# maua-maua-maua/maua

Hardware: AMD Instinct MI355X
Metric: frames/sec (whole node), 1024x1024 StyleGAN2 audio-reactive render (higher is better)
Workload: dtype bf16

## Files before the change

maua_amd/csrc/internal.h:

```cpp
#pragma once
#include "common.h"

namespace maua {

int launch_pack_rgb8(hipStream_t stream, const float* img, uint8_t* out, int B, int H, int W);
template <typename TI, typename TO>
int launch_nchw_to_nhwc(hipStream_t s, const void* x, void* y, int N, int C, int HW, int Cp);
template <typename TI, typename TO>
int launch_nhwc_to_nchw(hipStream_t s, const void* x, void* y, int N, int C, int HW, int Cp);

struct ConvArgs {
  const void* x;
  long x_bstride;
  const void* w;
  const float* s;
  const float* d;
  const float* noise;
  long noise_bstride;
  float noise_strength;
  const float* noise_scale;
  const float* bias;
  void* y;
  int B, H, W, Ci, Co, up;
  int act;
// ... 41 lines not shown

bool lowres_supported(int dtype, int Ci, int Co, int up, int H, int W);
void lowres_workspace(int dtype, int B, int H, int W, int Ci, int Co, int up, size_t* xm_bytes, size_t* ws_bytes);
int launch_modconv_lowres(hipStream_t stream, int dtype, const ConvArgs& a, void* xm, float* ws);

bool gather_conv_supported(int dtype, int Ci, int Co, int H, int W);
size_t gather_conv_workspace(int dtype, int B, int H, int W, int Ci, int Co);
int launch_conv_gather(hipStream_t stream, int dtype, const ConvArgs& a, float* ws);
int gather_conv_check(int dtype, const ConvArgs& a);
int gather_conv_ksplit(int dtype, int B, int H, int W, int Ci, int Co);

struct UnetConvRoute { int kernel; bool wide; int variant; };
UnetConvRoute unet_conv_route(int dtype, int route, int B, int H, int W, int Ci, int Co);

struct HiresArgs {
  const void* x;
  const void* w;
  const float* s;
  const float* d;
  const float* noise;
  long noise_bstride;
  float noise_strength;
  const float* noise_scale;
  const float* bias;
  void* y;
  int B, H, W, Ci, Co, up, act;
  float alpha, gain, clamp;
  const float* rgb_wmod;
  const float* rgb_bias;
  const float* rgb_prev;
  float* rgb_out;
  float rgb_clamp;
  float fir[16];
  uint8_t* rgb8_out;
  int rgb_skip_f32;
};
bool hires_supported(int dtype, int Ci, int Co, int up, int H, int W);
int launch_modconv_hires(hipStream_t stream, const HiresArgs& a, int dtype = MAUA_BF16);
bool upwalk_supported(int dtype, int Ci, int Co, int up, int H, int W);
size_t upwalk_weight_elems(int Co, int Ci);
int launch_upwalk(hipStream_t stream, const HiresArgs& a, int dtype = MAUA_BF16);
int launch_prep_upwalk_weights(hipStream_t stream, const float* w, void* wt, int Co, int Ci, int flip, int dtype = MAUA_BF16);
bool upwalk_fused_supported(int dtype, int Ci, int Cm, int H, int W);
int launch_upwalk_fused(hipStream_t stream, const HiresArgs& up, const HiresArgs& c1, int force_segs = 0, int narrow_ok = 1,
                        int dtype = MAUA_BF16);

int launch_prep_weights(hipStream_t stream, int dtype, const float* w, void* wt, float* wsq, int Co, int Ci, int k,
                        int up, int flip, int Cop, int Cip);
int launch_transpose_flip(hipStream_t stream, const float* w, float* w_t, int Co, int Ci, int kk);
int launch_f32_split_inplace(hipStream_t stream, void* w, long n_floats);

int launch_tconv2(hipStream_t stream, int dtype, const ConvArgs& a);
bool tconv_dma_supported(int dtype, int Ci, int Co, int H, int W);
int launch_tconv_dma(hipStream_t stream, const ConvArgs& a, int dtype = MAUA_BF16);
int launch_tconv_edges(hipStream_t stream, const ConvArgs& a, int dtype = MAUA_BF16);
int launch_prep_tconv_weights(hipStream_t stream, int dtype, const float* w, void* wt, int Co, int Ci, int flip);

struct UpfirArgs {
  const void* t;
  void* y;
  const float* d;
  const float* noise;
  long noise_bstride;
  float noise_strength;
  const float* noise_scale;
  const float* bias;
  const float* out_scale;
  int B, H, W, Co;
  int act;
  float alpha, gain, clamp;
};
int launch_upfir_epilogue(hipStream_t stream, int dtype, const UpfirArgs& a);
bool tconv_fir_supported(int dtype, int Ci, int Co, int H, int W);
int launch_tconv_fir(hipStream_t stream, const ConvArgs& a, const UpfirArgs& u, int dtype = MAUA_BF16, int walk = 1, int force_segs = 0);
size_t prepped_weight_elems(int k, int up, int Cop, int Cip);

struct LayerOperands { const void* x; const void* w; const float* s; const float* d; const float* bias; void* y; int B, H, W, Ci, Co, up; };
struct NoiseOperands { const float* noise; long bstride; float strength; const float* scale; };
struct Epilogue { int act; float alpha, gain, clamp; };
template <typename A>
inline void set_noise_args(A& a, const NoiseOperands& n) {
  a.noise = n.noise; a.noise_bstride = n.bstride; a.noise_strength = n.strength; a.noise_scale = n.scale;
}
template <typename A>
inline void set_epilogue_args(A& a, const Epilogue& e) {
  a.act = e.act; a.alpha = e.alpha; a.gain = e.gain; a.clamp = e.clamp;
}
template <typename A>
inline A layer_args(A a, const LayerOperands& l, const NoiseOperands& n, const Epilogue& e) {
  a.x = l.x; a.w = l.w; a.s = l.s; a.d = l.d; a.bias = l.bias; a.y = l.y;
  a.B = l.B; a.H = l.H; a.W = l.W; a.Ci = l.Ci; a.Co = l.Co; a.up = l.up;
  set_noise_args(a, n);
  set_epilogue_args(a, e);
  return a;
}
template <typename A>
inline void fuse_torgb_args(A& a, const float* wmod, const float* bias, const float* prev, float* out, float clamp, const float* fir16) {
  a.rgb_wmod = wmod; a.rgb_bias = bias; a.rgb_prev = prev; a.rgb_out = out; a.rgb_clamp = clamp;
  for (int i = 0; i < 16; i++) a.fir[i] = fir16[i];
}
inline void pack_u8_args(HiresArgs& a, uint8_t* rgb8_out, bool skip_f32) {
  a.rgb8_out = rgb8_out;
  a.rgb_skip_f32 = skip_f32;
}
inline ConvArgs tconv_args(const void* x, long x_bstride, const void* w, const float* s, void* t, int B, int H, int W, int Ci, int Co) {
  ConvArgs a{};
  a.x = x; a.x_bstride = x_bstride; a.w = w; a.s = s; a.y = t;
// ... 233 lines not shown
```

maua_amd/csrc/modconv_api.hip:

```cpp
#include <algorithm>
#include <cstring>

#include "common.h"
#include "internal.h"
#include "plain_conv.h"

namespace maua {
namespace {

enum { R_LOWRES = 0, R_GENERIC, R_DMA, R_HIRES, R_UPWALK, R_FUSED, R_WALKDONE, R_TFIR, R_TDMA, R_T2, R_UPFIR };

bool is_tconv(int r) { return r == R_TFIR || r == R_TDMA || r == R_T2; }
bool reads_premod(int r) { return r == R_TFIR || r == R_TDMA || r == R_DMA; }

LayerOperands operands(const maua_modconv_desc* d) {
  return LayerOperands{d->x, nullptr, d->s, d->d, d->bias, d->y, d->B, d->H, d->W, d->Ci, d->Co, d->up};
}
NoiseOperands noise_of(const maua_modconv_desc* d) { return NoiseOperands{d->noise, d->noise_bstride, d->noise_strength, d->noise_scale}; }
Epilogue epilogue_of(const maua_modconv_desc* d) { return Epilogue{d->act, d->alpha, d->gain, d->clamp}; }

template <typename A>
A desc_args(const maua_modconv_desc* d) {
  A a = layer_args(A{}, operands(d), noise_of(d), epilogue_of(d));
  if (d->rgb_out) {
// ... 135 lines not shown
  hipStream_t st = ctx->stream;
  if (route == R_UPWALK || route == R_FUSED) {
    if (int rc = launch_prep_upwalk_weights(st, d->w, base + o_w, d->Co, d->Ci, d->flip, dtype)) return rc;
  } else if (is_tconv(route)) {
    if (int rc = launch_prep_tconv_weights(st, dtype, d->w, base + o_w, d->Co, d->Ci, d->flip)) return rc;
  } else if (route != R_UPFIR) {
    if (int rc = launch_prep_weights(st, dtype, d->w, base + o_w, nullptr, d->Co, d->Ci, 3, d->up, d->up == 2 ? d->flip : 0, d->Co, d->Ci))
      return rc;
  }
  if (route == R_FUSED)
    if (int rc = launch_prep_weights(st, dtype, d1->w, base + o_w1, nullptr, d1->Co, d1->Ci, 3, 1, 0, d1->Co, d1->Ci)) return rc;
  const void* x = d->x;
  long x_bstride = d->x_bstride;
  if (reads_premod(route)) {
    if (int rc = launch_premod_nhwc(st, d->x, d->x_bstride, d->s, base + o_xm, d->B, (long)d->H * d->W, d->Ci, dtype)) return rc;
    x = base + o_xm;
    x_bstride = (long)d->H * d->W * d->Ci;
  }
  if (ones_bytes)
    if (int rc = launch_fill_ones(st, (float*)(base + o_ones), (long)d->B * d->Ci)) return rc;
  switch (route) {
    case R_LOWRES:
    case R_GENERIC:
    case R_DMA: {
      ConvArgs a = conv_args(d);
      a.x = x; a.x_bstride = x_bstride; a.w = base + o_w;
      if (route == R_DMA) a.s = nullptr;
      return route == R_LOWRES    ? launch_modconv_lowres(st, dtype, a, base + o_xm, (float*)(base + o_ws))
             : route == R_GENERIC ? launch_modconv3x3(st, dtype, a)
                                  : launch_modconv_dma(st, a, dtype);
    }
    case R_HIRES:
    case R_UPWALK:
    case R_FUSED: {
      HiresArgs a = hires_args(d);
      a.w = base + o_w;
      if (route == R_HIRES) return launch_modconv_hires(st, a, dtype);
      if (route == R_UPWALK) return launch_upwalk(st, a, dtype);
      HiresArgs f = hires_args(d1);
      f.x = nullptr; f.y = nullptr; f.w = base + o_w1;
      a.y = nullptr;
      return launch_upwalk_fused(st, a, f, force_segs, narrow_ok, dtype);
    }
    case R_TFIR:
    case R_TDMA:
    case R_T2: {
      void* t = d->t ? d->t : base + o_t;
      ConvArgs a = tconv_args(d);
      a.x = x; a.x_bstride = x_bstride; a.w = base + o_w; a.y = t;
      if (route != R_T2) a.s = (const float*)(base + o_ones);
      UpfirArgs u = upfir_args(d);
      if (route == R_TFIR) return launch_tconv_fir(st, a, u, dtype, force_segs >= 0, force_segs);
      if (route == R_TDMA) {
        if (int rc = launch_tconv_edges(st, a, dtype)) return rc;
        if (int rc = launch_tconv_dma(st, a, dtype)) return rc;
      } else if (int rc = launch_tconv2(st, dtype, a)) {
        return rc;
      }
      u.t = t;
      return launch_upfir_epilogue(st, dtype, u);
    }
    case R_UPFIR: {
      UpfirArgs u = upfir_args(d);
      u.t = d->x;
      return launch_upfir_epilogue(st, dtype, u);
    }
  }
  return MAUA_OK;
}

extern "C" int maua_torgb_ex(maua_ctx* ctx, const void* x, const float* wmod, const float* bias, const float* prev, float* out, int B,
                             int H, int W, int C, float clamp, int dtype) {
  MAUA_REQUIRE(ctx && x && wmod && bias && out, "maua_torgb_ex: NULL argument");
  MAUA_REQUIRE(B >= 0 && H > 0 && W > 0 && C > 0, "maua_torgb_ex: bad shape");
  MAUA_REQUIRE(!prev || (H % 2 == 0 && W % 2 == 0), "maua_torgb_ex: the skip image needs an even grid");
  RgbArgs r{};
  r.x = x; r.wmod = wmod; r.bias = bias; r.prev = prev; r.out = out; r.B = B; r.H = H; r.W = W; r.C = C; r.clamp = clamp;
  upsample_fir16(r.fir);
  return launch_torgb(ctx->stream, dtype, r);
}
```

maua_amd/csrc/modconv_tconv_dma.hip:

```cpp
#include "common.h"
#include "internal.h"
#include "mma.h"
#include "modconv_tconv.h"

namespace maua {

namespace {

constexpr int PTH = 8, PTW = 32;
constexpr int HW1 = PTW + 1, HPX = (PTH + 1) * HW1;
constexpr int KB = 64;
constexpr int HBUF = HPX * KB;
constexpr int WROWS = 9 * 32;
constexpr int WBUF = WROWS * KB;
constexpr int OFF_H = 2 * WBUF;
constexpr int NW = 4, NT = NW * 64;
constexpr int WJ = (WBUF / 1024 + NW - 1) / NW;
constexpr int HJ = (HPX * 4 + NT - 1) / NT;

}

template <typename F>
__global__ __launch_bounds__(NT, 2) void tconv_dma_kernel(ConvArgs a) {
  constexpr int ES = 128 * 2 + 16, PPP = 16;
  extern __shared__ __attribute__((aligned(1024))) char smem[];
  const unsigned lds0 = __builtin_amdgcn_readfirstlane(lds_off(smem));
  const int tid = threadIdx.x, lane = tid & 63;
  const int wave = __builtin_amdgcn_readfirstlane(tid >> 6);
  const int r = lane & 31, h = lane >> 5;
  const int tiles_x = a.W >> 5, tiles = tiles_x * (a.H >> 3), CB = a.Co >> 5;
  const int cbg = CB < 8 ? CB : 8, n_ts = tiles * a.B, per_group = ((n_ts + 7) >> 3) * 8 * cbg;
  const int L = blockIdx.x, grp = L / per_group, Lg = L - grp * per_group;
  const int xcd = Lg & 7, idx = Lg >> 3;
  const int cb = grp * cbg + idx % cbg, ts = (idx / cbg) * 8 + xcd;
  if (ts >= n_ts) return;
  const int b = ts / tiles, tile = ts - b * tiles;
  const int tyi = tile / tiles_x, txi = tile - tyi * tiles_x;
  const int ty0 = tyi * PTH, tx0 = txi * PTW;
  const char* xb = reinterpret_cast<const char*>(a.x) + (long)b * a.x_bstride * 2;
  const char* wp = reinterpret_cast<const char*>(a.w);

  unsigned hoff[HJ];
#pragma unroll
  for (int j = 0; j < HJ; j++) {
    const int P = (wave + NW * j) * 64 + lane;
    const int hp = P >> 2, q = (P & 3) ^ tconv_swz(hp);
    const int py = (hp * 1986) >> 16;
    const int px = hp - py * HW1;
    const int gy = ty0 - 1 + py, gx = tx0 - 1 + px;
    hoff[j] = 0xffffffffu;
    if (P < HPX * 4) {
      if (gy >= 0 && gx >= 0) {
        hoff[j] = (unsigned)(((gy * a.W + gx) * a.Ci + q * 8) * 2);
      } else {
        *reinterpret_cast<u32x4*>(smem + OFF_H + P * 16) = u32x4{0u, 0u, 0u, 0u};
        *reinterpret_cast<u32x4*>(smem + OFF_H + HBUF + P * 16) = u32x4{0u, 0u, 0u, 0u};
      }
    }
  }
  unsigned woff[WJ];
#pragma unroll
  for (int j = 0; j < WJ; j++) {
    const int ii = wave + NW * j;
    const int R = min(16 * ii + (lane >> 2), WROWS - 1);
    const int k = R >> 5, n = R & 31;
    const int q = (lane & 3) ^ tconv_swz(R);
    woff[j] = (unsigned)((((((kTconvSlot[k] * CB + cb) * 4 + kTconvCls[k]) * 32 + n) * a.Ci) + q * 8) * 2);
  }
#define TD_ISSUE(C_, BUF_)                                                                               \
  {                                                                                                      \
    const char* ws_ = wp + (long)(C_) * KB;                                                              \
    _Pragma("unroll") for (int j = 0; j < WJ; j++)                                                      \
      if (wave + NW * j < WBUF / 1024) dma16_s(ws_, woff[j], lds0 + (BUF_) * WBUF + (wave + NW * j) * 1024); \
    const char* xs_ = xb + (long)(C_) * KB;                                                              \
    _Pragma("unroll") for (int j = 0; j < HJ; j++)                                                      \
      if (hoff[j] != 0xffffffffu) dma16_s(xs_, hoff[j], lds0 + OFF_H + (BUF_) * HBUF + (wave + NW * j) * 1024); \
  }

  const int hp00 = (2 * wave) * HW1 + r;
  const unsigned b0 = (unsigned)(r * KB + ((tconv_swz(r) ^ h) << 4));
#define TD_A(HR_, Q1_, KS_, BUF_)                                                                                              \
  ({                                                                                                                           \
    const int hp_ = hpv + (HR_) * HW1 + (Q1_);                                                                                 \
    *reinterpret_cast<const u32x4*>(smem + ((OFF_H + (BUF_) * HBUF + hp_ * KB + ((tconv_swz(hp_) ^ h) << 4)) ^ ((KS_) << 5))); \
  })
#define TD_B(K_, KS_, BUF_) (*reinterpret_cast<const u32x4*>(smem + (BUF_) * WBUF + (K_) * 32 * KB + (b0 ^ ((KS_) << 5))))

  f32x16 acc[2][4];
#pragma unroll
  for (int R = 0; R < 2; R++)
#pragma unroll
    for (int c = 0; c < 4; c++)
#pragma unroll
      for (int e = 0; e < 16; e++) acc[R][c][e] = 0.f;

  const int n_chunks = a.Ci >> 5;
  TD_ISSUE(0, 0)
  if (n_chunks > 1) TD_ISSUE(1, 1)
  asm volatile("s_waitcnt vmcnt(0)" ::: "memory");
  __syncthreads();
  int hpv = hp00;
#define TD_STEP(KS_, BUF_)                                                                                            \
  {                                                                                                                   \
    u32x4 A00 = TD_A(0, 0, KS_, BUF_), A01 = TD_A(0, 1, KS_, BUF_);                  \
    u32x4 A10 = TD_A(1, 0, KS_, BUF_), A11 = TD_A(1, 1, KS_, BUF_);                                \
    u32x4 A20 = TD_A(2, 0, KS_, BUF_), A21 = TD_A(2, 1, KS_, BUF_);                                \
    {                                                                                                                 \
      const u32x4 B0 = TD_B(0, KS_, BUF_), B1 = TD_B(1, KS_, BUF_), B2 = TD_B(2, KS_, BUF_);                          \
      Mma<F>::step(acc[0][0], B0, A00); Mma<F>::step(acc[1][0], B0, A10);                            \
      Mma<F>::step(acc[0][1], B2, A01); Mma<F>::step(acc[1][1], B2, A11);                   \
      Mma<F>::step(acc[0][0], B1, A01); Mma<F>::step(acc[1][0], B1, A11);                   \
    }                                                                                                                 \
    {                                                                                                                 \
      const u32x4 B3 = TD_B(3, KS_, BUF_), B4 = TD_B(4, KS_, BUF_);                                                   \
      Mma<F>::step(acc[0][2], B4, A10); Mma<F>::step(acc[1][2], B4, A20);                   \
      Mma<F>::step(acc[0][0], B3, A10); Mma<F>::step(acc[1][0], B3, A20);                   \
    }                                                                                                                 \
    {                                                                                                                 \
      const u32x4 B5 = TD_B(5, KS_, BUF_), B6 = TD_B(6, KS_, BUF_), B7 = TD_B(7, KS_, BUF_), B8 = TD_B(8, KS_, BUF_); \
      Mma<F>::step(acc[0][3], B8, A11); Mma<F>::step(acc[1][3], B8, A21);                            \
      Mma<F>::step(acc[0][1], B6, A11); Mma<F>::step(acc[1][1], B6, A21);                                             \
      Mma<F>::step(acc[0][2], B7, A11); Mma<F>::step(acc[1][2], B7, A21);                                             \
      Mma<F>::step(acc[0][0], B5, A11); Mma<F>::step(acc[1][0], B5, A21);                                             \
    }                                                                                                                 \
  }
  for (int c = 0; c < n_chunks; c++) {
    const int buf = c & 1;
    asm volatile("" : "+v"(hpv));
    TD_STEP(0, buf)
    {
      u32x4 A00 = TD_A(0, 0, 1, buf), A01 = TD_A(0, 1, 1, buf), A10 = TD_A(1, 0, 1, buf), A11 = TD_A(1, 1, 1, buf);
      u32x4 A20 = TD_A(2, 0, 1, buf), A21 = TD_A(2, 1, 1, buf);
      const u32x4 B0 = TD_B(0, 1, buf), B1 = TD_B(1, 1, buf), B2 = TD_B(2, 1, buf), B3 = TD_B(3, 1, buf), B4 = TD_B(4, 1, buf);
      const u32x4 B5 = TD_B(5, 1, buf), B6 = TD_B(6, 1, buf), B7 = TD_B(7, 1, buf), B8 = TD_B(8, 1, buf);
      asm volatile("s_waitcnt vmcnt(0)" ::: "memory");
      __syncthreads();
      if (c + 2 < n_chunks) TD_ISSUE(c + 2, buf)
      Mma<F>::step(acc[0][0], B0, A00); Mma<F>::step(acc[1][0], B0, A10);
      Mma<F>::step(acc[0][1], B2, A01); Mma<F>::step(acc[1][1], B2, A11);
      Mma<F>::step(acc[0][0], B1, A01); Mma<F>::step(acc[1][0], B1, A11);
      Mma<F>::step(acc[0][2], B4, A10); Mma<F>::step(acc[1][2], B4, A20);
      Mma<F>::step(acc[0][0], B3, A10); Mma<F>::step(acc[1][0], B3, A20);
      Mma<F>::step(acc[0][3], B8, A11); Mma<F>::step(acc[1][3], B8, A21);
      Mma<F>::step(acc[0][1], B6, A11); Mma<F>::step(acc[1][1], B6, A21);
      Mma<F>::step(acc[0][2], B7, A11); Mma<F>::step(acc[1][2], B7, A21);
      Mma<F>::step(acc[0][0], B5, A11); Mma<F>::step(acc[1][0], B5, A21);
    }
  }
#undef TD_ISSUE
#undef TD_A
#undef TD_B
#undef TD_STEP

  const int Wt = 2 * a.W + 1, Ht = 2 * a.H + 1;
  __syncthreads();
  char* epi = smem;
#pragma unroll
  for (int R = 0; R < 2; R++) {
    const int m = (2 * wave + R) * 32 + r;
#pragma unroll
    for (int c = 0; c < 4; c++)
#pragma unroll
      for (int qd = 0; qd < 4; qd++)
        *reinterpret_cast<uint2*>(epi + m * ES + (c * 32 + 8 * qd + 4 * h) * 2) =
            make_uint2(Fmt16<F>::pack2(acc[R][c][qd * 4 + 0], acc[R][c][qd * 4 + 1]), Fmt16<F>::pack2(acc[R][c][qd * 4 + 2], acc[R][c][qd * 4 + 3]));
  }
  __syncthreads();
  char* yb = reinterpret_cast<char*>(a.y) + (long)b * Ht * Wt * a.Co * 2;
  for (int p = tid; p < PTH * PTW * PPP; p += NT) {
    const int mm = p / PPP, pc = p - mm * PPP;
    const int gy = ty0 + (mm >> 5), gx = tx0 + (mm & 31);
    const int nv = pc * 8, cls = nv >> 5, ch = nv & 31;
    const int oy = 2 * gy + (cls >> 1), ox = 2 * gx + (cls & 1);
    *reinterpret_cast<uint4*>(yb + (((long)oy * Wt + ox) * a.Co + cb * 32 + ch) * 2) =
        *reinterpret_cast<const uint4*>(epi + mm * ES + pc * 16);
  }
}

template <typename F>
__global__ __launch_bounds__(64) void tconv_edges_kernel(ConvArgs a, int row_tiles) {
  const int lane = threadIdx.x, r = lane & 31, h = lane >> 5;
  const int b = blockIdx.y, cb = blockIdx.z, CB = a.Co >> 5;
  const bool row_edge = (int)blockIdx.x < row_tiles;
  const int e0 = (row_edge ? (int)blockIdx.x : (int)blockIdx.x - row_tiles) * 32 + r;
  const uint16_t* xb = reinterpret_cast<const uint16_t*>(a.x) + (long)b * a.x_bstride;
  const uint16_t* wp = reinterpret_cast<const uint16_t*>(a.w);
  long x0 = -1, x1 = -1;
  if (row_edge) {
    if (e0 >= 1 && e0 <= a.W) x0 = ((long)(a.H - 1) * a.W + (e0 - 1)) * a.Ci;
    if (e0 < a.W) x1 = ((long)(a.H - 1) * a.W + e0) * a.Ci;
  } else {
    if (e0 >= 1 && e0 <= a.H - 1) x0 = ((long)(e0 - 1) * a.W + (a.W - 1)) * a.Ci;
    if (e0 < a.H) x1 = ((long)e0 * a.W + (a.W - 1)) * a.Ci;
  }
  const int s1 = row_edge ? 1 : 2, c2 = row_edge ? 1 : 2;
  const uint16_t* w0 = wp + ((((long)0 * CB + cb) * 4 + 0) * 32 + r) * a.Ci + 8 * h;
  const uint16_t* w1 = wp + ((((long)s1 * CB + cb) * 4 + 0) * 32 + r) * a.Ci + 8 * h;
  const uint16_t* w2 = wp + ((((long)s1 * CB + cb) * 4 + c2) * 32 + r) * a.Ci + 8 * h;
  f32x16 acc0, acc1;
#pragma unroll
  for (int e = 0; e < 16; e++) { acc0[e] = 0.f; acc1[e] = 0.f; }
  const u32x4 zero = u32x4{0u, 0u, 0u, 0u};
#pragma unroll 4
  for (int k = 0; k < a.Ci; k += 16) {
    const u32x4 A0 = *reinterpret_cast<const u32x4*>(w0 + k), A1 = *reinterpret_cast<const u32x4*>(w1 + k),
                A2 = *reinterpret_cast<const u32x4*>(w2 + k);
    const u32x4 X0 = x0 >= 0 ? *reinterpret_cast<const u32x4*>(xb + x0 + k + 8 * h) : zero;
    const u32x4 X1 = x1 >= 0 ? *reinterpret_cast<const u32x4*>(xb + x1 + k + 8 * h) : zero;
    Mma<F>::step(acc0, A0, X0);
    Mma<F>::step(acc1, A2, X1);
    Mma<F>::step(acc0, A1, X1);
  }
  const int Wt = 2 * a.W + 1, Ht = 2 * a.H + 1;
  uint16_t* yb = reinterpret_cast<uint16_t*>(a.y) + (long)b * Ht * Wt * a.Co + cb * 32 + 4 * h;
  long o0 = -1, o1 = -1;
  if (row_edge) {
    if (e0 <= a.W) o0 = ((long)(2 * a.H) * Wt + 2 * e0) * a.Co;
    if (e0 < a.W) o1 = ((long)(2 * a.H) * Wt + 2 * e0 + 1) * a.Co;
  } else if (e0 < a.H) {
    o0 = ((long)(2 * e0) * Wt + 2 * a.W) * a.Co;
    o1 = ((long)(2 * e0 + 1) * Wt + 2 * a.W) * a.Co;
  }
#pragma unroll
  for (int qd = 0; qd < 4; qd++) {
    if (o0 >= 0)
      *reinterpret_cast<uint2*>(yb + o0 + 8 * qd) = make_uint2(Fmt16<F>::pack2(acc0[qd * 4], acc0[qd * 4 + 1]), Fmt16<F>::pack2(acc0[qd * 4 + 2], acc0[qd * 4 + 3]));
    if (o1 >= 0)
      *reinterpret_cast<uint2*>(yb + o1 + 8 * qd) = make_uint2(Fmt16<F>::pack2(acc1[qd * 4], acc1[qd * 4 + 1]), Fmt16<F>::pack2(acc1[qd * 4 + 2], acc1[qd * 4 + 3]));
  }
}

int tconv_edges_check(const ConvArgs& a, int dtype) {
  MAUA_REQUIRE(dtype == MAUA_BF16 || dtype == MAUA_F16, "tconv_edges: unsupported dtype");
  MAUA_REQUIRE(a.Ci % 16 == 0 && a.Co % 32 == 0, "tconv_edges: Ci % 16, Co % 32");
  MAUA_REQUIRE(a.B <= 65535 && a.Co / 32 <= 65535, "tconv_edges: grid too large");
  return MAUA_OK;
}
int tconv_dma_check(const ConvArgs& a, int dtype) {
  MAUA_REQUIRE(tconv_dma_supported(dtype, a.Ci, a.Co, a.H, a.W), "tconv_dma: unsupported shape");
  const int tiles = (a.H / PTH) * (a.W / PTW), CB = a.Co / 32, cbg = CB < 8 ? CB : 8;
  MAUA_REQUIRE(CB % cbg == 0, "tconv_dma: channel blocks must split into groups of 8");
  const long n_ts = (long)tiles * a.B, grid = ((n_ts + 7) / 8) * 8 * cbg * (CB / cbg);
  MAUA_REQUIRE(grid < (1L << 31), "tconv_dma: grid too large");
  return MAUA_OK;
}

int launch_tconv_edges(hipStream_t stream, const ConvArgs& a, int dtype) {
  if (int rc = tconv_edges_check(a, dtype)) return rc;
  if (a.B == 0) return MAUA_OK;
  const int row_tiles = (a.W + 1 + 31) / 32, col_tiles = (a.H + 31) / 32;
  if (dtype == MAUA_F16)
    hipLaunchKernelGGL(tconv_edges_kernel<f16_t>, dim3(row_tiles + col_tiles, a.B, a.Co / 32), dim3(64), 0, stream, a, row_tiles);
  else
    hipLaunchKernelGGL(tconv_edges_kernel<bf16_t>, dim3(row_tiles + col_tiles, a.B, a.Co / 32), dim3(64), 0, stream, a, row_tiles);
  MAUA_HIP_CHECK(hipGetLastError());
  return MAUA_OK;
}

bool tconv_dma_supported(int dtype, int Ci, int Co, int H, int W) {
  return (dtype == MAUA_BF16 || dtype == MAUA_F16) && Ci % 32 == 0 && Co % 32 == 0 && H % PTH == 0 && W % PTW == 0 &&
         (long)H * W * Ci * 2 < (1L << 32) && 16L * Co * Ci * 2 < (1L << 32);
}

int launch_tconv_dma(hipStream_t stream, const ConvArgs& a, int dtype) {
  if (int rc = tconv_dma_check(a, dtype)) return rc;
  if (a.B == 0) return MAUA_OK;
  const int tiles = (a.H / PTH) * (a.W / PTW), CB = a.Co / 32, cbg = CB < 8 ? CB : 8;
  const long n_ts = (long)tiles * a.B, grid = ((n_ts + 7) / 8) * 8 * cbg * (CB / cbg);
  const size_t smem = std::max<size_t>((size_t)2 * WBUF + 2 * HBUF, (size_t)PTH * PTW * (128 * 2 + 16));
  if (dtype == MAUA_F16) {
    MAUA_HIP_CHECK(hipFuncSetAttribute((const void*)tconv_dma_kernel<f16_t>, hipFuncAttributeMaxDynamicSharedMemorySize, (int)smem));
    hipLaunchKernelGGL(tconv_dma_kernel<f16_t>, dim3((unsigned)grid), dim3(NT), smem, stream, a);
  } else {
    MAUA_HIP_CHECK(hipFuncSetAttribute((const void*)tconv_dma_kernel<bf16_t>, hipFuncAttributeMaxDynamicSharedMemorySize, (int)smem));
    hipLaunchKernelGGL(tconv_dma_kernel<bf16_t>, dim3((unsigned)grid), dim3(NT), smem, stream, a);
  }
  MAUA_HIP_CHECK(hipGetLastError());
  return MAUA_OK;
}

}
```

maua_amd/csrc/synth.hip:

```cpp
#include <cmath>
#include <cstring>
#include <string>
#include <vector>

#include "common.h"
#include "internal.h"
#include "plain_conv.h"

using namespace maua;

namespace {

struct ConvLayer {
  int block, which;
  int Ci, Co, res, up, w_index;
  int ih = 0, iw = 0;
  int oh = 0, ow = 0;
  int fh = 0, fw = 0;
  float* affine_w = nullptr;
  float* affine_b = nullptr;
  float* bias = nullptr;
  float* noise_const = nullptr;
  float noise_strength = 0.f;
  void* wt = nullptr;
  void* wt_t = nullptr;
  void* wt_h = nullptr;
  float* wsq = nullptr;
  float* s = nullptr;
  float* d = nullptr;
  void* feat = nullptr;
};
struct RgbLayer {
  int block, C, res, w_index;
  int h = 0, w = 0;
  float* affine_w = nullptr;
  float* affine_b = nullptr;
  float* wrgb = nullptr;
  float* bias = nullptr;
  float* s = nullptr;
  float* wmod = nullptr;
};

template <typename T>
int dev_alloc(T** p, size_t n) {
  MAUA_HIP_CHECK(hipMalloc((void**)p, n * sizeof(T)));
  return MAUA_OK;
}

}

struct maua_synth {
  maua_ctx* ctx;
  int res, w_dim, channel_base, channel_max, dtype, nv_compat;
  int nblocks, num_ws;
  size_t esize;
  std::vector<ConvLayer> convs;
  std::vector<RgbLayer> rgbs;
  void* const_x = nullptr;
  int keep_features = 0;
  int lowres = 1;
  int use_hires = 1;
  int upwalk = 2;
  int walk_segs = 0;
  int walk_narrow = 1;
  int fuse_torgb = 1;
  int tconv_up = 1;
  int tconv_fir = 256;
  int tconv_walk = 1;
  const float* nz_scales = nullptr;
  long nz_scale_stride = 0;
  int dma_conv = 1;
  int dual_store = 1;
  int tconv_dma = 1;
  UnitStyles ones;
  void* xm = nullptr;
  void* tbuf = nullptr;
  void* lowres_xm = nullptr;
  float* lowres_ws = nullptr;
  int rs_layer = -1, rs_mode = 0, rs_th = 0, rs_tw = 0, rs_pl = 0, rs_pr = 0, rs_pt = 0, rs_pb = 0, rs_how = 3;
  float rs_value = 0.f;
  float* rs_noise = nullptr;
  void* const_rs = nullptr;
  float* rgb_tmp[2] = {nullptr, nullptr};
  int out_h = 0, out_w = 0;
  int warp_layer[3] = {-1, -1, -1};
  const float* warp_minv[3] = {nullptr, nullptr, nullptr};
  int profile = 0;
  std::vector<hipEvent_t> ev;
  size_t ev_used = 0;
  std::vector<size_t> ev_fwd_start;
  int bcap = 0;
  void* act[2] = {nullptr, nullptr};
  float* img[2] = {nullptr, nullptr};
  StyleLayer* style_table_dev = nullptr;
  float fir[16];
};

static void prof_mark(maua_synth* n) {
  if (!n->profile || n->ev_used >= (1u << 16)) return;
  if (n->ev_used == n->ev.size()) {
    hipEvent_t e;
    if (hipEventCreate(&e) != hipSuccess) return;
    n->ev.push_back(e);
  }
  hipEventRecord(n->ev[n->ev_used++], n->ctx->stream);
}

static int channels_for(int res, int base, int maxc) { return std::min(base / res, maxc); }

static bool lowres_fits(const maua_synth* n, const ConvLayer& c) {
  return lowres_supported(n->dtype, c.Ci, c.Co, c.up, c.ih, c.iw);
}
static bool tconv_dma_fits(const maua_synth* n, const ConvLayer& c) {
  return c.up == 2 && tconv_dma_supported(n->dtype, c.Ci, c.Co, c.ih, c.iw);
}

static void compute_dims(maua_synth* n) {
  int h = 4, w = 4;
  if (n->rs_layer == 0) { h = n->rs_th; w = n->rs_tw; }
  size_t li = 0;
  for (int blk = 0; blk < n->nblocks; blk++) {
    const int nconv = blk == 0 ? 1 : 2;
    for (int k = 0; k < nconv; k++, li++) {
      ConvLayer& c = n->convs[li];
      c.ih = h; c.iw = w;
      c.oh = h * c.up; c.ow = w * c.up;
// ... 355 lines not shown
    MAUA_HIP_CHECK(hipMemcpy(n->rs_noise, fill_noise_host, cnt * sizeof(float), hipMemcpyHostToDevice));
  }
  compute_dims(n);
  free_workspace(n);
  for (size_t i = 0; i < n->convs.size(); i++) {
    ConvLayer& c = n->convs[i];
    if (c.oh != before[i].oh || c.ow != before[i].ow) {
      hipFree(c.noise_const);
      c.noise_const = nullptr;
      MAUA_HIP_CHECK(hipMalloc((void**)&c.noise_const, (size_t)c.oh * c.ow * sizeof(float)));
      MAUA_HIP_CHECK(hipMemset(c.noise_const, 0, (size_t)c.oh * c.ow * sizeof(float)));
    }
  }
  return MAUA_OK;
}

int maua_synth_set_warp(maua_synth* n, int slot, int layer, const float* inv_matrices_dev) {
  MAUA_REQUIRE(n, "maua_synth_set_warp: net is NULL");
  MAUA_REQUIRE(slot >= 0 && slot < 3, "maua_synth_set_warp: slot must be 0..2");
  MAUA_REQUIRE(layer >= 1 && layer <= (int)n->convs.size(), "maua_synth_set_warp: layer must name a synthesis layer (1-based index into layer_names)");
  n->warp_layer[slot] = inv_matrices_dev ? layer : -1;
  n->warp_minv[slot] = inv_matrices_dev;
  return MAUA_OK;
}

int maua_synth_layer_size(const maua_synth* n, int layer, int* h, int* w) {
  MAUA_REQUIRE(n && h && w, "maua_synth_layer_size: NULL argument");
  MAUA_REQUIRE(layer >= -1 && layer < (int)n->convs.size(), "maua_synth_layer_size: no such layer");
  if (layer < 0) { *h = n->out_h; *w = n->out_w; }
  else { *h = n->convs[layer].oh; *w = n->convs[layer].ow; }
  return MAUA_OK;
}

int maua_synth_set_option(maua_synth* n, const char* key, int value) {
  MAUA_REQUIRE(n && key, "maua_synth_set_option: NULL argument");
  if (!strcmp(key, "profile")) {
    n->profile = value;
    n->ev_used = 0;
    n->ev_fwd_start.clear();
    return MAUA_OK;
  }
  if (!strcmp(key, "keep_features")) {
    if (n->keep_features != value) {
      MAUA_HIP_CHECK(hipStreamSynchronize(n->ctx->stream));
      free_workspace(n);
      n->keep_features = value;
    }
    return MAUA_OK;
  }
  static const std::pair<const char*, int maua_synth::*> routing[] = {
      {"lowres", &maua_synth::lowres},         {"use_hires", &maua_synth::use_hires}, {"upwalk", &maua_synth::upwalk},
      {"walk_segs", &maua_synth::walk_segs},   {"walk_narrow", &maua_synth::walk_narrow},
      {"fuse_torgb", &maua_synth::fuse_torgb}, {"tconv_up", &maua_synth::tconv_up},   {"tconv_fir", &maua_synth::tconv_fir},
      {"tconv_walk", &maua_synth::tconv_walk},
      {"tconv_dma", &maua_synth::tconv_dma},   {"dma_conv", &maua_synth::dma_conv},   {"dual_store", &maua_synth::dual_store}};
  for (const auto& o : routing)
    if (!strcmp(key, o.first)) {
      n->*o.second = value;
      return MAUA_OK;
    }
  return fail(std::string("maua_synth_set_option: unknown option ") + key);
}

static thread_local hipMemcpyKind g_load_kind = hipMemcpyHostToDevice;

static int upload(float* dst, const float* host, size_t count, size_t expect, const char* name) {
  if (count != expect)
    return fail(std::string("maua_synth_load: ") + name + ": expected " + std::to_string(expect) + " values, got " +
                std::to_string(count));
  MAUA_HIP_CHECK(hipMemcpy(dst, host, count * sizeof(float), g_load_kind));
  return MAUA_OK;
}

int maua_synth_load(maua_synth* n, const char* name, const float* host, size_t count) {
  MAUA_REQUIRE(n && name && host, "maua_synth_load: NULL argument");
  std::string s(name);
  int blk = -1, pos = 0;
  if (sscanf(name, "bs.%d.%n", &blk, &pos) < 1 || blk < 0 || blk >= n->nblocks || pos == 0)
    return fail("maua_synth_load: unknown parameter name: " + s);
  std::string rest = s.substr(pos);
  hipStream_t st = n->ctx->stream;
  auto check_filter = [&]() -> int {
    if (count != 16) return fail("maua_synth_load: " + s + ": only the 4x4 [1,3,3,1] resample filter is supported");
    const float t[4] = {1, 3, 3, 1};
    for (int u = 0; u < 4; u++)
      for (int v = 0; v < 4; v++)
        if (std::fabs(host[u * 4 + v] - t[u] * t[v] / 64.f) > 1e-6f)
          return fail("maua_synth_load: " + s + ": only the 4x4 [1,3,3,1] resample filter is supported");
    return MAUA_OK;
  };
  if (rest == "resample_filter") return check_filter();
  if (rest == "const") {
    if (blk != 0) return fail("maua_synth_load: only block 0 has a const input");
    int C = n->convs[0].Ci;
    if (count != (size_t)C * 16) return fail("maua_synth_load: bs.0.const: wrong size");
    DevTemp tmp;
    if (int rc = tmp.stage(host, count, g_load_kind)) return rc;
    int rc = n->dtype == MAUA_BF16   ? launch_nchw_to_nhwc<float, bf16_t>(st, tmp.p, n->const_x, 1, C, 16, C)
             : n->dtype == MAUA_F16 ? launch_nchw_to_nhwc<float, f16_t>(st, tmp.p, n->const_x, 1, C, 16, C)
                                    : launch_nchw_to_nhwc<float, float>(st, tmp.p, n->const_x, 1, C, 16, C);
    hipStreamSynchronize(st);
    return rc;
  }
  size_t dot = rest.find('.');
  if (dot == std::string::npos) return fail("maua_synth_load: unknown parameter name: " + s);
  std::string mod = rest.substr(0, dot), par = rest.substr(dot + 1);
  if (mod == "torgb") {
// ... 116 lines not shown
      switch (s.route) {
        case Route::Lowres:
        case Route::Generic:
        case Route::DmaConv1: {
          ConvArgs a = layer_args(ConvArgs{}, li, x, y);
          a.x_bstride = x_bstride;
          a.out_scale = next_s;
          if (s.dual) a.y_scaled = n->xm;
          if (s.rgb) fuse_torgb(a);
          if (s.route == Route::DmaConv1) a.s = nullptr;
          if (int rc = s.route == Route::Lowres    ? launch_modconv_lowres(st, n->dtype, a, n->lowres_xm, n->lowres_ws)
                       : s.route == Route::Generic ? launch_modconv3x3(st, n->dtype, a)
                                                   : launch_modconv_dma(st, a, n->dtype))
            return rc;
          break;
        }
        case Route::Hires:
        case Route::Upwalk:
        case Route::FusedWalk: {
          HiresArgs a = layer_args(HiresArgs{}, li, x, s.skip_store ? nullptr : y);
          if (s.rgb) fuse_torgb(a);
          if (s.rgb8) pack_u8(a);
          if (s.route != Route::Hires) a.w = c.wt_h;
          if (s.route != Route::FusedWalk) {
            if (int rc = s.route == Route::Hires ? launch_modconv_hires(st, a, n->dtype) : launch_upwalk(st, a, n->dtype)) return rc;
            break;
          }
          HiresArgs f = layer_args(HiresArgs{}, li + 1, nullptr, nullptr);
          fuse_torgb(f);
          if (plan.conv[li + 1].rgb8) pack_u8(f);
          if (int rc = launch_upwalk_fused(st, a, f, n->walk_segs, n->walk_narrow, n->dtype)) return rc;
          break;
        }
        case Route::WalkDone:
          break;
        case Route::TconvFir:
        case Route::TconvDma:
        case Route::Tconv2: {
          ConvArgs a = tconv_args(x, x_bstride, c.wt_t, c.s, n->tbuf, B, c.ih, c.iw, c.Ci, c.Co);
          UpfirArgs u = upfir_args(y, c.d, c.bias, next_s, B, c.ih, c.iw, c.Co, layer_noise(li), lrelu_epilogue());
          if (s.src == Src::PremodPass)
            if (int rc = launch_premod_nhwc(st, x, x_bstride, c.s, n->xm, B, (long)c.ih * c.iw, c.Ci, n->dtype)) return rc;
          if (s.src == Src::PremodPass || s.src == Src::Xm) {
            a.x = n->xm;
            a.x_bstride = (long)c.ih * c.iw * c.Ci;
          }
          if (reads_premod(s.route)) a.s = n->ones.p;
          if (s.route == Route::TconvFir) {
            if (int rc = launch_tconv_fir(st, a, u, n->dtype, n->tconv_walk, 0)) return rc;
            prof_mark(n);
            break;
          }
          if (s.route == Route::TconvDma) {
            if (int rc = launch_tconv_edges(st, a, n->dtype)) return rc;
            if (int rc = launch_tconv_dma(st, a, n->dtype)) return rc;
          } else if (int rc = launch_tconv2(st, n->dtype, a)) {
            return rc;
          }
          prof_mark(n);
          u.t = n->tbuf;
          if (int rc = launch_upfir_epilogue(st, n->dtype, u)) return rc;
          break;
        }
      }
      prof_mark(n);
      x = y;
      x_bstride = (long)c.oh * c.ow * c.Co;
      cur ^= 1;
      if (hooked) {
        void* dst = n->keep_features ? c.feat : n->act[cur];
        if (int rc = resize_feat(x, x_bstride, B, c.oh, c.ow, c.Co, dst)) return rc;
        x = dst;
        x_bstride = (long)c.fh * c.fw * c.Co;
        cur ^= 1;
      }
      for (int wsl = 0; wsl < 3; wsl++) {
        if (n->warp_layer[wsl] != (int)li + 1 || !n->warp_minv[wsl]) continue;
        void* dst = n->act[cur];
        if (dst == x) dst = n->act[cur ^ 1];
        if (int rc = launch_warp_affine_nhwc(st, n->dtype, x, dst, n->warp_minv[wsl], B, c.fh, c.fw, c.Co)) return rc;
        if (n->keep_features) {
          MAUA_HIP_CHECK(hipMemcpyAsync(c.feat, dst, (size_t)B * c.fh * c.fw * c.Co * n->esize, hipMemcpyDeviceToDevice, st));
        } else {
          x = dst;
          cur = (dst == n->act[0]) ? 1 : 0;
        }
      }
    }
    if (plan.rgb[blk] != RgbRoute::Fused) {
      const bool hook = plan.rgb[blk] == RgbRoute::Hook;
      RgbArgs r{};
      r.x = x; r.wmod = g.wmod; r.bias = g.bias; r.prev = hook ? nullptr : prev_img;
      r.out = hook ? n->rgb_tmp[0] : rgb_out; r.B = B; r.H = g.h; r.W = g.w; r.C = g.C; r.clamp = 256.f;
      memcpy(r.fir, n->fir, sizeof(r.fir));
      if (int rc = launch_torgb(st, n->dtype, r)) return rc;
      if (hook) {
        const ConvLayer& hc = n->convs[n->rs_layer - 1];
        const int nh = hc.oh, nw = hc.ow;
        ResizeArgs inv{};
        inv.x = n->rgb_tmp[0]; inv.x_bstride = 3L * g.h * g.w; inv.y = n->rgb_tmp[1]; inv.B = B; inv.H = g.h; inv.W = g.w;
        inv.C = 3; inv.oh = nh; inv.ow = nw; inv.mode = n->rs_mode; inv.pl = -n->rs_pl; inv.pt = -n->rs_pt;
        inv.how = MAUA_PAD_CONSTANT; inv.value = 0.f; inv.noise = nullptr;
        if (int rc = launch_resize2d(st, MAUA_F32, false, inv)) return rc;
        const float* native = n->rgb_tmp[1];
        if (prev_img) {
          if (int rc = launch_skip_add(st, n->rgb_tmp[1], prev_img, n->rgb_tmp[0], B, nh, nw, n->fir)) return rc;
          native = n->rgb_tmp[0];
        }
// ... 85 lines not shown
```

Baseline: 4626.

## Fold transposed-conv edge rows and columns into the DMA tconv kernel

Removes the separate tconv_edges kernel launch by having the last-row and last-column tiles of the DMA transposed-conv kernel compute the border outputs with extra MMA steps inside the main K loop. The kernel is templated on an EDGES flag and specialises the loop per tile so interior tiles keep the original instruction stream. Edge waves carry two extra accumulators and write them out directly. This saves one launch and a pass over input and weights per upsampling layer, at the cost of load imbalance on edge tiles and higher register pressure.

```diff
diff --git a/maua_amd/csrc/internal.h b/maua_amd/csrc/internal.h
--- a/maua_amd/csrc/internal.h
+++ b/maua_amd/csrc/internal.h
@@ -117,7 +117,7 @@
 
 int launch_tconv2(hipStream_t stream, int dtype, const ConvArgs& a);
 bool tconv_dma_supported(int dtype, int Ci, int Co, int H, int W);
-int launch_tconv_dma(hipStream_t stream, const ConvArgs& a, int dtype = MAUA_BF16);
+int launch_tconv_dma(hipStream_t stream, const ConvArgs& a, int dtype = MAUA_BF16, bool edges = true);
 int launch_tconv_edges(hipStream_t stream, const ConvArgs& a, int dtype = MAUA_BF16);
 int launch_prep_tconv_weights(hipStream_t stream, int dtype, const float* w, void* wt, int Co, int Ci, int flip);
 
diff --git a/maua_amd/csrc/modconv_api.hip b/maua_amd/csrc/modconv_api.hip
--- a/maua_amd/csrc/modconv_api.hip
+++ b/maua_amd/csrc/modconv_api.hip
@@ -211,8 +211,9 @@
       UpfirArgs u = upfir_args(d);
       if (route == R_TFIR) return launch_tconv_fir(st, a, u, dtype, force_segs >= 0, force_segs);
       if (route == R_TDMA) {
-        if (int rc = launch_tconv_edges(st, a, dtype)) return rc;
-        if (int rc = launch_tconv_dma(st, a, dtype)) return rc;
+        if (force_segs < 0)
+          if (int rc = launch_tconv_edges(st, a, dtype)) return rc;
+        if (int rc = launch_tconv_dma(st, a, dtype, force_segs >= 0)) return rc;
       } else if (int rc = launch_tconv2(st, dtype, a)) {
         return rc;
       }
diff --git a/maua_amd/csrc/modconv_tconv_dma.hip b/maua_amd/csrc/modconv_tconv_dma.hip
--- a/maua_amd/csrc/modconv_tconv_dma.hip
+++ b/maua_amd/csrc/modconv_tconv_dma.hip
@@ -20,7 +20,7 @@
 
 }
 
-template <typename F>
+template <typename F, bool EDGES>
 __global__ __launch_bounds__(NT, 2) void tconv_dma_kernel(ConvArgs a) {
   constexpr int ES = 128 * 2 + 16, PPP = 16;
   extern __shared__ __attribute__((aligned(1024))) char smem[];
@@ -37,6 +37,8 @@
   const int b = ts / tiles, tile = ts - b * tiles;
   const int tyi = tile / tiles_x, txi = tile - tyi * tiles_x;
   const int ty0 = tyi * PTH, tx0 = txi * PTW;
+  const bool row_edge = EDGES && wave == NW - 1 && tyi == (a.H >> 3) - 1;
+  const bool col_edge = EDGES && wave == 0 && txi == tiles_x - 1;
   const char* xb = reinterpret_cast<const char*>(a.x) + (long)b * a.x_bstride * 2;
   const char* wp = reinterpret_cast<const char*>(a.w);
 
@@ -86,7 +88,24 @@
   })
 #define TD_B(K_, KS_, BUF_) (*reinterpret_cast<const u32x4*>(smem + (BUF_) * WBUF + (K_) * 32 * KB + (b0 ^ ((KS_) << 5))))
 
-  f32x16 acc[2][4];
+  const int hpx0 = min(r, PTH) * HW1 + PTW, hpx1 = min(r + 1, PTH) * HW1 + PTW;
+  const unsigned xo0 = (unsigned)(OFF_H + hpx0 * KB + ((tconv_swz(hpx0) ^ h) << 4));
+  const unsigned xo1 = (unsigned)(OFF_H + hpx1 * KB + ((tconv_swz(hpx1) ^ h) << 4));
+#define TD_X(XO_, KS_, BUF_) (*reinterpret_cast<const u32x4*>(smem + (((XO_) + (BUF_) * HBUF) ^ ((KS_) << 5))))
+#define TD_COL(KS_, BUF_)                                                                                \
+  if constexpr (COL) {                                                                                   \
+    const u32x4 X0 = TD_X(xo0, KS_, BUF_);                                                               \
+    u32x4 X1 = TD_X(xo1, KS_, BUF_);                                                                     \
+    if (r >= PTH) X1 = u32x4{0u, 0u, 0u, 0u};                                                            \
+    const u32x4 C0 = TD_B(0, KS_, BUF_), C3 = TD_B(3, KS_, BUF_), C4 = TD_B(4, KS_, BUF_);               \
+    Mma<F>::step(e0, C0, X0); Mma<F>::step(e1, C4, X1); Mma<F>::step(e0, C3, X1);                        \
+  }
+#define TD_ROW(B0_, B1_, B2_, A20_, A21_)                                                                \
+  if constexpr (ROW) { Mma<F>::step(e0, B0_, A20_); Mma<F>::step(e1, B2_, A21_); Mma<F>::step(e0, B1_, A21_); }
+
+  f32x16 acc[2][4], e0, e1;
+#pragma unroll
+  for (int e = 0; e < 16; e++) { e0[e] = 0.f; e1[e] = 0.f; }
 #pragma unroll
   for (int R = 0; R < 2; R++)
 #pragma unroll
@@ -102,6 +121,7 @@
   int hpv = hp00;
 #define TD_STEP(KS_, BUF_)                                                                                            \
   {                                                                                                                   \
+    TD_COL(KS_, BUF_)                                                                                                 \
     u32x4 A00 = TD_A(0, 0, KS_, BUF_), A01 = TD_A(0, 1, KS_, BUF_);                  \
     u32x4 A10 = TD_A(1, 0, KS_, BUF_), A11 = TD_A(1, 1, KS_, BUF_);                                \
     u32x4 A20 = TD_A(2, 0, KS_, BUF_), A21 = TD_A(2, 1, KS_, BUF_);                                \
@@ -110,6 +130,7 @@
       Mma<F>::step(acc[0][0], B0, A00); Mma<F>::step(acc[1][0], B0, A10);                            \
       Mma<F>::step(acc[0][1], B2, A01); Mma<F>::step(acc[1][1], B2, A11);                   \
       Mma<F>::step(acc[0][0], B1, A01); Mma<F>::step(acc[1][0], B1, A11);                   \
+      TD_ROW(B0, B1, B2, A20, A21)                                                                \
     }                                                                                                                 \
     {                                                                                                                 \
       const u32x4 B3 = TD_B(3, KS_, BUF_), B4 = TD_B(4, KS_, BUF_);                                                   \
@@ -124,11 +145,14 @@
       Mma<F>::step(acc[0][0], B5, A11); Mma<F>::step(acc[1][0], B5, A21);                                             \
     }                                                                                                                 \
   }
+  auto k_loop = [&](auto col_, auto row_) __attribute__((always_inline)) {
+  constexpr bool COL = decltype(col_)::value, ROW = decltype(row_)::value;
   for (int c = 0; c < n_chunks; c++) {
     const int buf = c & 1;
     asm volatile("" : "+v"(hpv));
     TD_STEP(0, buf)
     {
+      TD_COL(1, buf)
       u32x4 A00 = TD_A(0, 0, 1, buf), A01 = TD_A(0, 1, 1, buf), A10 = TD_A(1, 0, 1, buf), A11 = TD_A(1, 1, 1, buf);
       u32x4 A20 = TD_A(2, 0, 1, buf), A21 = TD_A(2, 1, 1, buf);
       const u32x4 B0 = TD_B(0, 1, buf), B1 = TD_B(1, 1, buf), B2 = TD_B(2, 1, buf), B3 = TD_B(3, 1, buf), B4 = TD_B(4, 1, buf);
@@ -139,6 +163,7 @@
       Mma<F>::step(acc[0][0], B0, A00); Mma<F>::step(acc[1][0], B0, A10);
       Mma<F>::step(acc[0][1], B2, A01); Mma<F>::step(acc[1][1], B2, A11);
       Mma<F>::step(acc[0][0], B1, A01); Mma<F>::step(acc[1][0], B1, A11);
+      TD_ROW(B0, B1, B2, A20, A21)
       Mma<F>::step(acc[0][2], B4, A10); Mma<F>::step(acc[1][2], B4, A20);
       Mma<F>::step(acc[0][0], B3, A10); Mma<F>::step(acc[1][0], B3, A20);
       Mma<F>::step(acc[0][3], B8, A11); Mma<F>::step(acc[1][3], B8, A21);
@@ -147,12 +172,41 @@
       Mma<F>::step(acc[0][0], B5, A11); Mma<F>::step(acc[1][0], B5, A21);
     }
   }
+  };
+  if (EDGES && row_edge) k_loop(std::false_type{}, std::true_type{});
+  else if (EDGES && col_edge) k_loop(std::true_type{}, std::false_type{});
+  else k_loop(std::false_type{}, std::false_type{});
 #undef TD_ISSUE
 #undef TD_A
 #undef TD_B
 #undef TD_STEP
+#undef TD_X
+#undef TD_COL
+#undef TD_ROW
 
   const int Wt = 2 * a.W + 1, Ht = 2 * a.H + 1;
+  char* yb = reinterpret_cast<char*>(a.y) + (long)b * Ht * Wt * a.Co * 2;
+  if (EDGES && (row_edge || col_edge)) {
+    long o0 = -1, o1 = -1;
+    if (row_edge) {
+      o0 = ((long)(2 * a.H) * Wt + 2 * (tx0 + r)) * a.Co;
+      o1 = o0 + a.Co;
+    } else if (r < PTH) {
+      o0 = ((long)(2 * (ty0 + r)) * Wt + 2 * a.W) * a.Co;
+      o1 = o0 + (long)Wt * a.Co;
+    } else if (r == PTH && ty0 + PTH == a.H) {
+      o0 = ((long)(2 * a.H) * Wt + 2 * a.W) * a.Co;
+    }
+    uint16_t* ye = reinterpret_cast<uint16_t*>(yb) + cb * 32 + 4 * h;
+#pragma unroll
+    for (int qd = 0; qd < 4; qd++) {
+      if (o0 >= 0)
+        *reinterpret_cast<uint2*>(ye + o0 + 8 * qd) = make_uint2(Fmt16<F>::pack2(e0[qd * 4], e0[qd * 4 + 1]), Fmt16<F>::pack2(e0[qd * 4 + 2], e0[qd * 4 + 3]));
+      if (o1 >= 0)
+        *reinterpret_cast<uint2*>(ye + o1 + 8 * qd) = make_uint2(Fmt16<F>::pack2(e1[qd * 4], e1[qd * 4 + 1]), Fmt16<F>::pack2(e1[qd * 4 + 2], e1[qd * 4 + 3]));
+    }
+  }
+
   __syncthreads();
   char* epi = smem;
 #pragma unroll
@@ -166,7 +220,6 @@
             make_uint2(Fmt16<F>::pack2(acc[R][c][qd * 4 + 0], acc[R][c][qd * 4 + 1]), Fmt16<F>::pack2(acc[R][c][qd * 4 + 2], acc[R][c][qd * 4 + 3]));
   }
   __syncthreads();
-  char* yb = reinterpret_cast<char*>(a.y) + (long)b * Ht * Wt * a.Co * 2;
   for (int p = tid; p < PTH * PTW * PPP; p += NT) {
     const int mm = p / PPP, pc = p - mm * PPP;
     const int gy = ty0 + (mm >> 5), gx = tx0 + (mm & 31);
@@ -262,19 +315,26 @@
          (long)H * W * Ci * 2 < (1L << 32) && 16L * Co * Ci * 2 < (1L << 32);
 }
 
-int launch_tconv_dma(hipStream_t stream, const ConvArgs& a, int dtype) {
+template <typename F, bool EDGES>
+static int tconv_dma_launch(hipStream_t stream, const ConvArgs& a, unsigned grid, size_t smem) {
+  MAUA_HIP_CHECK(hipFuncSetAttribute((const void*)tconv_dma_kernel<F, EDGES>, hipFuncAttributeMaxDynamicSharedMemorySize, (int)smem));
+  hipLaunchKernelGGL((tconv_dma_kernel<F, EDGES>), dim3(grid), dim3(NT), smem, stream, a);
+  return MAUA_OK;
+}
+
+int launch_tconv_dma(hipStream_t stream, const ConvArgs& a, int dtype, bool edges) {
+  if (edges)
+    if (int rc = tconv_edges_check(a, dtype)) return rc;
   if (int rc = tconv_dma_check(a, dtype)) return rc;
   if (a.B == 0) return MAUA_OK;
   const int tiles = (a.H / PTH) * (a.W / PTW), CB = a.Co / 32, cbg = CB < 8 ? CB : 8;
-  const long n_ts = (long)tiles * a.B, grid = ((n_ts + 7) / 8) * 8 * cbg * (CB / cbg);
+  const long n_ts = (long)tiles * a.B;
+  const unsigned grid = (unsigned)(((n_ts + 7) / 8) * 8 * cbg * (CB / cbg));
   const size_t smem = std::max<size_t>((size_t)2 * WBUF + 2 * HBUF, (size_t)PTH * PTW * (128 * 2 + 16));
-  if (dtype == MAUA_F16) {
-    MAUA_HIP_CHECK(hipFuncSetAttribute((const void*)tconv_dma_kernel<f16_t>, hipFuncAttributeMaxDynamicSharedMemorySize, (int)smem));
-    hipLaunchKernelGGL(tconv_dma_kernel<f16_t>, dim3((unsigned)grid), dim3(NT), smem, stream, a);
-  } else {
-    MAUA_HIP_CHECK(hipFuncSetAttribute((const void*)tconv_dma_kernel<bf16_t>, hipFuncAttributeMaxDynamicSharedMemorySize, (int)smem));
-    hipLaunchKernelGGL(tconv_dma_kernel<bf16_t>, dim3((unsigned)grid), dim3(NT), smem, stream, a);
-  }
+  const bool f16 = dtype == MAUA_F16;
+  if (int rc = edges ? (f16 ? tconv_dma_launch<f16_t, true>(stream, a, grid, smem) : tconv_dma_launch<bf16_t, true>(stream, a, grid, smem))
+                     : (f16 ? tconv_dma_launch<f16_t, false>(stream, a, grid, smem) : tconv_dma_launch<bf16_t, false>(stream, a, grid, smem)))
+    return rc;
   MAUA_HIP_CHECK(hipGetLastError());
   return MAUA_OK;
 }
diff --git a/maua_amd/csrc/synth.hip b/maua_amd/csrc/synth.hip
--- a/maua_amd/csrc/synth.hip
+++ b/maua_amd/csrc/synth.hip
@@ -72,6 +72,7 @@
   int dma_conv = 1;
   int dual_store = 1;
   int tconv_dma = 1;
+  int tconv_edges_fold = 1;
   UnitStyles ones;
   void* xm = nullptr;
   void* tbuf = nullptr;
@@ -533,7 +534,7 @@
       {"lowres", &maua_synth::lowres},         {"use_hires", &maua_synth::use_hires}, {"upwalk", &maua_synth::upwalk},
       {"walk_segs", &maua_synth::walk_segs},   {"walk_narrow", &maua_synth::walk_narrow},
       {"fuse_torgb", &maua_synth::fuse_torgb}, {"tconv_up", &maua_synth::tconv_up},   {"tconv_fir", &maua_synth::tconv_fir},
-      {"tconv_walk", &maua_synth::tconv_walk},
+      {"tconv_walk", &maua_synth::tconv_walk}, {"tconv_edges_fold", &maua_synth::tconv_edges_fold},
       {"tconv_dma", &maua_synth::tconv_dma},   {"dma_conv", &maua_synth::dma_conv},   {"dual_store", &maua_synth::dual_store}};
   for (const auto& o : routing)
     if (!strcmp(key, o.first)) {
@@ -756,8 +757,9 @@
             break;
           }
           if (s.route == Route::TconvDma) {
-            if (int rc = launch_tconv_edges(st, a, n->dtype)) return rc;
-            if (int rc = launch_tconv_dma(st, a, n->dtype)) return rc;
+            if (!n->tconv_edges_fold)
+              if (int rc = launch_tconv_edges(st, a, n->dtype)) return rc;
+            if (int rc = launch_tconv_dma(st, a, n->dtype, n->tconv_edges_fold != 0)) return rc;
           } else if (int rc = launch_tconv2(st, n->dtype, a)) {
             return rc;
           }
```

New measurement: 4644 (median of 6 runs). About the same (+0.4%).
